# liuyuan-pal/Gen6D

Hardware: NVIDIA H100
Metric: poses/sec end-to-end (128^2 crop, 64 refs, 3 refine iters) (higher is better)
Workload: dtype f32

## Files before the change

gen6d_b200/_lib.py:

```python
import ctypes as C
import os
import re

HERE = os.path.dirname(os.path.abspath(__file__))
LIB_PATH = os.path.join(HERE, 'libgen6d_b200.so')
HEADER_PATH = os.path.join(os.path.dirname(HERE), 'include', 'gen6d_b200.h')

G6D_DET_MAX_SCALES = 8
G6D_GLUE_MAX_OBJECTS = 16
G6D_DET_MAX_INSTANCES = 16
G6D_DET_MAX_PEAK_RADIUS = 3
G6D_ATTENTION_MAX_SMEM_FLOATS = 12288 - 32
G6D_FRAMES_MAX = 1024
G6D_FRAME_RGB, G6D_FRAME_NV12 = 0, 1
PRO_NONE, PRO_AFFINE, PRO_AFFINE_RELU, PRO_CORR = 0, 1, 2, 3
ACT_NONE, ACT_RELU, ACT_LEAKY01 = 0, 1, 2
TC_TF32, TC_F16 = 0, 1
TC_PRENORM, TC_REUSE_IM2COL, TC_FOLD_SPLITS = 1, 4, 32


class ConvDesc(C.Structure):
    _fields_ = [(n, C.c_int) for n in ('B', 'D', 'H', 'W', 'Cin', 'in_cstride', 'in_coff', 'Cout', 'kd', 'kh', 'kw',
                                       'stride', 'pd', 'ph', 'pw', 'Do', 'Ho', 'Wo', 'out_cstride', 'out_coff',
                                       'prologue')] + [('group_rows', C.c_longlong), ('act', C.c_int), ('max_chain_k', C.c_int)]


class DetMaps(C.Structure):
    _fields_ = [('n_scales', C.c_int), ('rfn', C.c_int), ('hs', C.c_int), ('ws', C.c_int),
                ('map', (C.c_void_p * 3) * G6D_DET_MAX_SCALES),
                ('H', (C.c_int * 3) * G6D_DET_MAX_SCALES), ('W', (C.c_int * 3) * G6D_DET_MAX_SCALES),
                ('mu', C.c_float * 3), ('inv_sigma', C.c_float * 3), ('clip', C.c_float)]


class GlueCamera(C.Structure):
    _fields_ = [('K', C.c_double * 9), ('Kinv', C.c_double * 9), ('f', C.c_double), ('f_sq', C.c_double)]


class GlueRefs(C.Structure):
    _fields_ = [('poses', C.c_void_p), ('cen', C.c_void_p), ('f', C.c_void_p), ('dist', C.c_void_p), ('center', C.c_double * 3)]


class GlueViews(C.Structure):
    _fields_ = [('poses', C.c_void_p), ('R_look', C.c_void_p), ('RlookR', C.c_void_p), ('f', C.c_void_p), ('Kinv', C.c_void_p),
                ('src', C.c_void_p), ('rows', C.c_void_p), ('cols', C.c_void_p), ('even_idx', C.c_void_p), ('even_dirs', C.c_void_p),
                ('n_views', C.c_int), ('n_even', C.c_int), ('ref_num', C.c_int), ('size', C.c_int),
                ('norm_scale', C.c_double), ('norm_offset', C.c_float * 3), ('size_scale', C.c_float)]

# ... 136 lines not shown
```

gen6d_b200/csrc/conv_ffma.cu:

```cuda
#include "common.cuh"

namespace g6d {

struct ConvP {
    const float* x; const float* w; const float* bias; const float* ps; const float* pb;
    float* y; float* ws;
    int B, D, H, W, Cin, ics, ico, Cout, ldw, kd, kh, kw, stride, pd, ph, pw, Do, Ho, Wo, ocs, oco, pro, act;
    long long group_rows;
    int M, K, ktiles, splits, kt_per_split;
};

constexpr int BM = 128, BK = 16, NT = 256;

__device__ __forceinline__ float act_apply(float v, int act) {
    if (act == G6D_ACT_RELU) return fmaxf(v, 0.f);
    if (act == G6D_ACT_LEAKY01) return v > 0.f ? v : 0.1f * v;
    return v;
}

template <int TN>
__global__ void __launch_bounds__(NT, 2) conv_ffma_kernel(const ConvP p) {
    constexpr int BN = 16 * TN;
    constexpr int HN = BN / 2;
    constexpr int B_F4 = (BK * BN / 4);
// ... 286 lines not shown
    }
}

static int fill_params(const g6d_conv_desc* d, ConvP& p) {
    G6D_REQUIRE(d != nullptr, "g6d_conv: null desc");
    G6D_REQUIRE(d->B > 0 && d->D > 0 && d->H > 0 && d->W > 0 && d->Cin > 0 && d->Cout > 0, "g6d_conv: bad dims");
    G6D_REQUIRE(d->kd > 0 && d->kh > 0 && d->kw > 0 && d->stride > 0, "g6d_conv: bad kernel/stride");
    G6D_REQUIRE((d->Cin & 3) == 0 && (d->in_cstride & 3) == 0 && (d->in_coff & 3) == 0,
                "g6d_conv: Cin (%d), in_cstride (%d), in_coff (%d) must be multiples of 4", d->Cin, d->in_cstride,
                d->in_coff);
    G6D_REQUIRE(d->in_coff + d->Cin <= d->in_cstride, "g6d_conv: input channel slice out of row");
    G6D_REQUIRE(d->out_coff + d->Cout <= d->out_cstride, "g6d_conv: output channel slice out of row");
    const int Do = (d->D + 2 * d->pd - d->kd) / d->stride + 1;
    const int Ho = (d->H + 2 * d->ph - d->kh) / d->stride + 1;
    const int Wo = (d->W + 2 * d->pw - d->kw) / d->stride + 1;
    G6D_REQUIRE(Do == d->Do && Ho == d->Ho && Wo == d->Wo, "g6d_conv: output dims mismatch (%d,%d,%d) vs (%d,%d,%d)",
                d->Do, d->Ho, d->Wo, Do, Ho, Wo);
    G6D_REQUIRE(d->prologue >= 0 && d->prologue <= 3 && d->act >= 0 && d->act <= 2, "g6d_conv: bad prologue/act");
    if (d->prologue == G6D_PRO_AFFINE || d->prologue == G6D_PRO_AFFINE_RELU)
        G6D_REQUIRE(d->group_rows > 0, "g6d_conv: group_rows must be > 0 for affine prologue");
    const long long M = (long long)d->B * Do * Ho * Wo;
    const long long K = (long long)d->kd * d->kh * d->kw * d->Cin;
    G6D_REQUIRE(M < (1ll << 31) && K < (1ll << 31), "g6d_conv: problem too large");
    p.B = d->B; p.D = d->D; p.H = d->H; p.W = d->W; p.Cin = d->Cin; p.ics = d->in_cstride; p.ico = d->in_coff;
    p.Cout = d->Cout; p.ldw = (d->Cout + 3) & ~3; p.kd = d->kd; p.kh = d->kh; p.kw = d->kw; p.stride = d->stride;
    p.pd = d->pd; p.ph = d->ph; p.pw = d->pw; p.Do = Do; p.Ho = Ho; p.Wo = Wo; p.ocs = d->out_cstride;
    p.oco = d->out_coff; p.pro = d->prologue; p.act = d->act; p.group_rows = d->group_rows > 0 ? d->group_rows : 1;
    p.M = (int)M; p.K = (int)K; p.ktiles = (int)((K + BK - 1) / BK);
    const int bn = d->Cout > 64 ? 128 : (d->Cout > 32 ? 64 : 32);
    const long long ctas = (long long)ceil_div(M, BM) * ceil_div(d->Cout, bn);
    int splits = 1;
    if (ctas < kNumSMs && p.ktiles >= 16) {
        splits = (int)((2 * kNumSMs + ctas - 1) / ctas);
        splits = splits > p.ktiles / 8 ? p.ktiles / 8 : splits;
        splits = splits > 64 ? 64 : splits;
        splits = splits < 1 ? 1 : splits;
    }
    p.kt_per_split = (p.ktiles + splits - 1) / splits;
    p.splits = (p.ktiles + p.kt_per_split - 1) / p.kt_per_split;
    return G6D_OK;
}

}

using namespace g6d;

extern "C" long long g6d_conv_workspace_bytes(const g6d_conv_desc* desc) {
    ConvP p{};
    if (fill_params(desc, p) != G6D_OK) return -1;
    return p.splits > 1 ? (long long)p.splits * p.M * p.Cout * (long long)sizeof(float) : 0;
}

extern "C" int g6d_conv(const g6d_conv_desc* desc, const float* x, const float* w, const float* bias,
// ... 132 lines not shown
```

gen6d_b200/csrc/conv_tc.cu:

```cuda
#include <cuda_fp16.h>
#include <string.h>

#include "tc_common.cuh"

namespace g6d {

constexpr int TC_BM = 128;
constexpr int TC_PRODUCER_WARPS = 8;
constexpr int TC_CONSUMER_WARPS = 8;
constexpr int TC_THREADS = (TC_PRODUCER_WARPS + TC_CONSUMER_WARPS) * 32;
constexpr int TC_ISSUER = TC_PRODUCER_WARPS * 32;
constexpr int TC_PRODUCER_REGS = 96, TC_CONSUMER_REGS = 160;
static_assert(TC_PRODUCER_WARPS * TC_PRODUCER_REGS + TC_CONSUMER_WARPS * TC_CONSUMER_REGS <= 65536 / 32, "register file of one SM");
constexpr int TC_FOLD_PRODUCER_REGS = 40, TC_FOLD_CONSUMER_REGS = 216;
static_assert(TC_PRODUCER_WARPS * TC_FOLD_PRODUCER_REGS + TC_CONSUMER_WARPS * TC_FOLD_CONSUMER_REGS <= 65536 / 32, "register file of one SM");
static_assert(TC_BM == 64 * (TC_CONSUMER_WARPS / 4), "one 64-row wgmma tile per consumer warpgroup");
constexpr int TC_MAX_K_PER_CHAIN = 2048;

template <int KIND> struct KindCfg;
template <> struct KindCfg<G6D_TC_TF32> {
    static constexpr int BK = 32;
    static constexpr int NV = 1;
    static constexpr float CROSS = 1.f;
};
// ... 865 lines not shown
           (long long)d->D * d->H * d->W < (1ll << 30) && d->group_rows < (1ll << 31);
}

static int fill_tc_params(const g6d_conv_desc* d, int kind, ConvTcP& p) {
    G6D_REQUIRE(d != nullptr, "g6d_conv_tc: null desc");
    G6D_REQUIRE(kind == G6D_TC_TF32 || kind == G6D_TC_F16, "g6d_conv_tc: bad operand kind %d", kind);
    G6D_REQUIRE(d->B > 0 && d->D > 0 && d->H > 0 && d->W > 0 && d->Cin > 0, "g6d_conv_tc: bad dims");
    G6D_REQUIRE(d->Cout >= 16, "g6d_conv_tc: Cout (%d) must be at least 16", d->Cout);
    G6D_REQUIRE(d->kd > 0 && d->kh > 0 && d->kw > 0 && d->stride > 0, "g6d_conv_tc: bad kernel/stride");
    const int bk = kind_bk(kind);
    G6D_REQUIRE((d->Cin % bk) == 0, "g6d_conv_tc: Cin (%d) must be a multiple of %d", d->Cin, bk);
    G6D_REQUIRE((d->in_cstride & 3) == 0 && (d->in_coff & 3) == 0, "g6d_conv_tc: in_cstride/in_coff must be multiples of 4");
    G6D_REQUIRE(d->in_coff + d->Cin <= d->in_cstride, "g6d_conv_tc: input channel slice out of row");
    G6D_REQUIRE(d->out_coff + d->Cout <= d->out_cstride, "g6d_conv_tc: output channel slice out of row");
    G6D_REQUIRE(tc2_dims_ok(d), "g6d_conv_tc: spatial extent too large for the tensor-core kernel");
    const int Do = (d->D + 2 * d->pd - d->kd) / d->stride + 1;
    const int Ho = (d->H + 2 * d->ph - d->kh) / d->stride + 1;
    const int Wo = (d->W + 2 * d->pw - d->kw) / d->stride + 1;
    G6D_REQUIRE(Do > 0 && Ho > 0 && Wo > 0 && Do == d->Do && Ho == d->Ho && Wo == d->Wo, "g6d_conv_tc: output dims mismatch");
    G6D_REQUIRE(d->prologue >= 0 && d->prologue <= 3 && d->act >= 0 && d->act <= 2, "g6d_conv_tc: bad prologue/act");
    const long long M = (long long)d->B * Do * Ho * Wo;
    const long long K = (long long)d->kd * d->kh * d->kw * d->Cin;
    G6D_REQUIRE(M < (1ll << 31) && K < (1ll << 31), "g6d_conv_tc: problem too large");
    p.B = d->B; p.D = d->D; p.H = d->H; p.W = d->W; p.Cin = d->Cin; p.ics = d->in_cstride; p.ico = d->in_coff;
    p.Cout = d->Cout; p.kd = d->kd; p.kh = d->kh; p.kw = d->kw; p.stride = d->stride; p.pd = d->pd; p.ph = d->ph;
    p.pw = d->pw; p.Do = Do; p.Ho = Ho; p.Wo = Wo; p.ocs = d->out_cstride; p.oco = d->out_coff; p.pro = d->prologue;
    p.act = d->act; p.group_rows = d->group_rows > 0 ? d->group_rows : 1;
    p.M = (int)M; p.K = (int)K; p.kblocks = (int)(K / bk);
    const int bn = tc_block_n(d->Cout);
    const long long ctas = (long long)ceil_div(M, TC_BM) * ceil_div(d->Cout, bn);
    const int min_kb = 256 / bk;
    int splits = 1;
    if (ctas < kNumSMs && p.kblocks >= 2 * min_kb) {
        splits = (int)(kNumSMs / ctas);
        splits = splits > p.kblocks / min_kb ? p.kblocks / min_kb : splits;
        splits = splits < 1 ? 1 : splits;
    }
    const int nmain = tc_nmain(bn);
    const int chain = d->max_chain_k > 0 ? d->max_chain_k * nmain : (K > TC_MAX_K_PER_CHAIN ? TC_MAX_K_PER_CHAIN * nmain : 0);
    const int max_kb = chain > bk ? chain / bk : 1;
    const int min_splits = chain > 0 ? (p.kblocks + max_kb - 1) / max_kb : 1;
    splits = splits < min_splits ? min_splits : splits;
    splits = splits > 64 ? 64 : splits;
    p.kb_per_split = (p.kblocks + splits - 1) / splits;
    p.splits = (p.kblocks + p.kb_per_split - 1) / p.kb_per_split;
    return G6D_OK;
}

template <int BN, int KIND, bool FOLD, bool XR>
static int launch_tc2(const ConvTcP& p, const CUtensorMap& mh, const CUtensorMap& ml, const CUtensorMap& ma, cudaStream_t st) {
    constexpr int SMEM = XR ? Tc2XrCfg<BN>::SMEM_BYTES : Tc2Cfg<BN>::SMEM_BYTES;
    static bool configured = false;
    if (!configured) {
// ... 307 lines not shown
    const int rows = TC_BM + (d->kh - 1) * Wp + d->kw - 1;
    const int budget = 220 * 1024;
    const int b_stage = 2 * bn * 128;
    {
        const long long tiles = ((long long)Ho * Wp + TC_BM - 1) / TC_BM;
        if ((long long)Ho * Wo * 100 < tiles * TC_BM * 60) return false;
    }
    const long long a_stage = 2ll * ((rows + 7) / 8 * 8) * 128;
    const int tab_bytes = 4 * rows;
    int a_st = 2, b_st = 3;
    long long used = a_st * a_stage + b_st * b_stage + tab_bytes + 2048;
    if (used > budget) return false;
    while (b_st < 4 && used + b_stage <= budget) { ++b_st; used += b_stage; }
    while (a_st < 4 && used + a_stage <= budget) { ++a_st; used += a_stage; }
    p.B = d->B; p.D = d->D; p.H = d->H; p.W = d->W; p.Cin = d->Cin; p.ics = d->in_cstride; p.ico = d->in_coff;
    p.Cout = d->Cout; p.kd = d->kd; p.kh = d->kh; p.kw = d->kw; p.pd = d->pd; p.ph = d->ph; p.pw = d->pw;
    p.Do = Do; p.Ho = Ho; p.Wo = Wo; p.ocs = d->out_cstride; p.oco = d->out_coff; p.pro = d->prologue; p.act = d->act;
    p.group_rows = d->group_rows > 0 ? d->group_rows : 1;
    p.Wp = Wp; p.tiles_per_plane = (Ho * Wp + TC_BM - 1) / TC_BM;
    p.seg_rows = rows; p.rows_pad = (rows + 7) / 8 * 8; p.cblocks = d->Cin / kind_bk(kind);
    p.M = d->B * Do * Ho * Wo;
    p.a_stages = a_st; p.b_stages = b_st;
    *smem_bytes = (int)(a_st * a_stage) + b_st * b_stage + 256 + tab_bytes + 1024 + 64;
    const long long ctas = (long long)d->B * Do * p.tiles_per_plane * ((d->Cout + bn - 1) / bn);
    const long long K = (long long)d->Cin * d->kd * d->kh * d->kw;
    int splits = 1;
    if (ctas < kNumSMs && p.cblocks >= 2) splits = (int)((kNumSMs + ctas - 1) / ctas);
    const int nmain = tc_nmain(bn);
    const long long chain = d->max_chain_k > 0 ? (long long)d->max_chain_k * nmain : (K > TC_MAX_K_PER_CHAIN ? TC_MAX_K_PER_CHAIN * nmain : 0);
    if (chain > 0) { const int ms = (int)((K + chain - 1) / chain); splits = splits < ms ? ms : splits; }
    splits = splits > p.cblocks ? p.cblocks : splits;
    splits = splits < 1 ? 1 : splits;
    p.cb_per_split = (p.cblocks + splits - 1) / splits;
    p.splits = (p.cblocks + p.cb_per_split - 1) / p.cb_per_split;
    return true;
}

__global__ void __launch_bounds__(256) flat_moments_kernel(const float* __restrict__ y, int ocs, int oco, int Cout, int Ho, int Wo,
                                                           int Wp, int slices_per_plane, double* __restrict__ stats,
                                                           long long stats_rows) {
    __shared__ double red[8][4][4];
    const int warp = threadIdx.x >> 5, lane = threadIdx.x & 31;
    const long long m_plane = (long long)blockIdx.x * Ho * Wo;
    const int n0 = 8 * blockIdx.y + 2 * (lane & 3);
    double acc[4] = {0.0, 0.0, 0.0, 0.0};
    for (int sl = warp; sl < slices_per_plane; sl += 8) {
        const int f = sl * 16 + (lane >> 2);
// ... 327 lines not shown
```

gen6d_b200/network/selector.py:

```python
from dataclasses import dataclass

import numpy as np
import torch

from .. import ops
from .backbone import pack_vgg, vgg_v1
from .base import Branches, PackedModule, linear_as_conv
from .params import SEL_TOWER_POST, SEL_TOWERS, VGG11BNParams, selector_modules

IN_EPS = 1e-5


class LocalComm:
    rank, world, capturable = 0, 1, True

    def all_reduce_sum(self, t):
        return t

    def all_gather_cat(self, t, dim=0):
        return t

    def shard_range(self, n):
        return 0, n


FEAT_PAD = 516


@dataclass
class SelectorRefs:
    feats_cache: list
    sums: list
    pose_embed: torch.Tensor
    shape: tuple
    rfn_total: int


class ViewpointSelector(PackedModule):
    default_cfg = {'selector_angle_num': 5}

    def __init__(self, cfg):
        self.cfg = {**self.default_cfg, **cfg}
        super().__init__()
        self.backbone = VGG11BNParams()
        for name, mod in selector_modules(self.cfg['selector_angle_num']).items():
            setattr(self, name, mod)
        self.refs = None
        self.comm = LocalComm()

# ... 77 lines not shown
        x = vp.to(self.device).reshape(rfn, 1, 1, 4)
        for i, pc in enumerate(p['vpe']):
            x = ops.conv(x, pc, act=ops.ACT_RELU if i < 2 else ops.ACT_NONE)
        return SelectorRefs(feats_cache, sums, x.reshape(rfn, 512), (rfn, an), rfn_total)

    @staticmethod
    def s2_counters_for(refs, device):
        return torch.zeros(3 * refs.shape[0] * refs.shape[1], device=device, dtype=torch.int32)

    def comm_stats(self):
        return dict(getattr(self.comm, 'calls', {}))

    def _s2_counters(self):
        n = 3 * self.ref_shape[0] * self.ref_shape[1]
        c = self.__dict__.get('_s2_done')
        if c is None or c.numel() != n or c.device != self.device:
            c = torch.zeros(n, device=self.device, dtype=torch.int32)
            self.__dict__['_s2_done'] = c
        return c

    def _finalize(self, ws, rows_total):
        return ops.instnorm_finalize(self.comm.all_reduce_sum(ws), rows_total, IN_EPS)

    def _tower(self, level, ref, scale, shift, cat_buf, S, refs):
        convs = self.packed()['towers'][level]
        x, pro, ps, pb = ref, ops.PRO_CORR, scale, shift
        for i, (pc, post) in enumerate(convs):
            last = i + 1 == len(convs)
            if last:
                ops.conv(x, pc, prologue=pro, pro_scale=ps, pro_shift=pb, group_rows=S, out=cat_buf, out_coff=256 * level,
                         prenorm=True, reuse_im2col=True, fold_splits=True)
                break
            rows = x.shape[0] * x.shape[1] * x.shape[2]
            y, ws = ops.conv(x, pc, prologue=pro, pro_scale=ps, pro_shift=pb, group_rows=S, stats_rows=rows, prenorm=True,
                             reuse_im2col=True, fold_splits=True)
            ps, pb = self._finalize(ws, rows // refs.shape[0] * refs.rfn_total)
            pro = ops.PRO_AFFINE_RELU if 'r' in post else ops.PRO_AFFINE
            x = ops.maxpool2x2(y) if 'p' in post else y

    def _towers_sharded(self, q_feats, cat_buf, S, S_total, refs):
        towers = self.packed()['towers']
        nbr = 3 if self.comm.capturable else 1
        state, keep = [], []
        for l, (q, ref, (s1, s2)) in enumerate(zip(q_feats, refs.feats_cache, refs.sums)):
            h, w, c = q.shape
            scale, shift = ops.sel_corr_prologue(q.reshape(h * w, c), s1, s2, S_total, IN_EPS)
            state.append({'x': ref, 'pro': ops.PRO_CORR, 'ps': scale, 'pb': shift, 'i': 0})
        for _ in range(max(len(t) for t in towers)):
            br = Branches(nbr)
            pend = []
            for l, st in enumerate(state):
                convs = towers[l]
                if st['i'] >= len(convs):
                    continue
                pc, post = convs[st['i']]
                last = st['i'] + 1 == len(convs)

                def step(l=l, st=st, pc=pc, last=last):
                    if last:
                        ops.conv(st['x'], pc, prologue=st['pro'], pro_scale=st['ps'], pro_shift=st['pb'], group_rows=S,
                                 out=cat_buf, out_coff=256 * l, prenorm=True, reuse_im2col=True,
                                 fold_splits=True)
                        return None
                    rows = st['x'].shape[0] * st['x'].shape[1] * st['x'].shape[2]
                    return ops.conv(st['x'], pc, prologue=st['pro'], pro_scale=st['ps'], pro_shift=st['pb'], group_rows=S,
                                    stats_rows=rows, prenorm=True, reuse_im2col=True, fold_splits=True) + (rows,)
                res = br.run(l, step)
                st['i'] += 1
                if res is not None:
                    pend.append((st, post, res))
            br.join()
            if not pend:
                continue
            flat = torch.cat([ws.reshape(-1) for _, _, (_, ws, _) in pend]) if len(pend) > 1 else pend[0][2][1].reshape(-1)
            flat = self.comm.all_reduce_sum(flat)
            o = 0
            for st, post, (y, ws, rows) in pend:
                n = ws.numel()
                ps, pb = ops.instnorm_finalize(flat[o:o + n].reshape(ws.shape), rows // refs.shape[0] * refs.rfn_total, IN_EPS)
                o += n
                keep.append((y, ws))
                st['ps'], st['pb'] = ps, pb
                st['pro'] = ops.PRO_AFFINE_RELU if 'r' in post else ops.PRO_AFFINE
                st['x'] = ops.maxpool2x2(y) if 'p' in post else y

    def _select_one(self, q_feats, refs=None, counters=None):
        p = self.packed()
        if refs is None:
            refs, counters = self.refs, self._s2_counters()
        rfn, an = refs.shape
        S = rfn * an
        S_total = refs.rfn_total * an
        if counters is None or counters.numel() != 3 * S:
            raise ValueError('_select_one: a reference record other than the module\'s needs its own S2 counters [3*S]')
        dev = self.device
        cat_buf = torch.empty(S, 4, 4, 768, device=dev, dtype=torch.float32)
        feats = torch.empty(S, FEAT_PAD, device=dev, dtype=torch.float32)
        scores = ops.sel_corr_score3([r.reshape(S, -1, r.shape[-1]) for r in refs.feats_cache],
                                     [q.reshape(-1, q.shape[-1]) for q in q_feats], counters=counters)
        if self.comm.world == 1:
            br = Branches(3)
            keep = []

            def one_level(l, q, ref, s1, s2):
                h, w, c = q.shape
                scale, shift = ops.sel_corr_prologue(q.reshape(h * w, c), s1, s2, S_total, IN_EPS)
                keep.append((scale, shift))
                self._tower(l, ref, scale, shift, cat_buf, S, refs)

            for l, (q, ref, (s1, s2)) in enumerate(zip(q_feats, refs.feats_cache, refs.sums)):
                br.run(l, lambda l=l, q=q, ref=ref, s1=s1, s2=s2: one_level(l, q, ref, s1, s2))
            br.join()
        else:
            self._towers_sharded(q_feats, cat_buf, S, S_total, refs)
        y, ws = ops.conv(cat_buf, p['cf0'], stats_rows=S * 16)
        ps, pb = self._finalize(ws, S_total * 16)
        y = ops.avgpool_affine(y.reshape(S * 16, 512), 16, ps, pb, rows_per_group=S * 16, act=ops.ACT_RELU)
        ops.conv(y.reshape(S, 1, 1, 512), p['cf3'], out=feats.reshape(S, 1, 1, FEAT_PAD), out_coff=0)
        if self.comm.world == 1:
            ops.sel_vp_norm(scores, feats, 512, IN_EPS)
        else:
            all_scores = self.comm.all_gather_cat(scores, dim=1).contiguous()
            tmp = torch.empty(S_total, 4, device=dev, dtype=torch.float32)
            ops.sel_vp_norm(all_scores, tmp, 0, IN_EPS)
            r0, _ = self.comm.shard_range(refs.rfn_total)
            feats[:, 512:516] = tmp[r0 * an:r0 * an + S]
        x = ops.conv(feats.reshape(S, 1, 1, FEAT_PAD), p['sp0'], act=ops.ACT_RELU)
        x = ops.conv(x, p['sp2']).reshape(rfn, an, 512)
        sf = ops.sel_max_angle_add(x, refs.pose_embed)
        sf = self.comm.all_gather_cat(sf, dim=0).contiguous()
        rfn_local, rfn = rfn, refs.rfn_total
        for att, (m0, m3) in zip(p['atts'], p['mlps']):
            x4 = sf.reshape(rfn, 1, 1, 512)
            qv = ops.conv(x4, att['conv_query']).reshape(rfn, 512)
            kv = ops.conv(x4, att['conv_key']).reshape(rfn, 512)
            vv = ops.conv(x4, att['conv_feats']).reshape(rfn, 512)
            msg = ops.attention(qv, kv, vv, heads=8, head_major=True)
            msg = ops.conv(msg.reshape(rfn, 1, 1, 512), att['conv_merge']).reshape(rfn, 512)
            msg = ops.layernorm(msg, att['ln_w'], att['ln_b'], 1e-5)
            y = ops.conv(torch.cat([sf, msg], 1).reshape(rfn, 1, 1, 1024), m0)
            ps, pb = ops.instnorm_stats(y, rows_per_group=rfn, eps=IN_EPS)
            y = ops.conv(y, m3, prologue=ops.PRO_AFFINE_RELU, pro_scale=ps, pro_shift=pb, group_rows=rfn)
            ps, pb = ops.instnorm_stats(y, rows_per_group=rfn, eps=IN_EPS)
            y = ops.affine_act(y.reshape(rfn, 512), ps, pb, rows_per_group=rfn, act=ops.ACT_RELU)
            sf = ops.add(y, sf)
        x = ops.conv(sf.reshape(rfn, 1, 1, 512), p['score_predict'][0], act=ops.ACT_RELU)
        logits = ops.conv(x, p['score_predict'][1]).reshape(rfn)
        x = feats.reshape(rfn_local, 1, 1, an * FEAT_PAD)
        for i, pc in enumerate(p['angle_predict']):
            x = ops.conv(x, pc, act=ops.ACT_RELU if i < 2 else ops.ACT_NONE)
        angles = self.comm.all_gather_cat(x.reshape(rfn_local), dim=0)
        return logits, angles, scores

    def _select_nhwc(self, que_norm4):
        if self.ref_feats_cache is None:
            raise RuntimeError('ViewpointSelector: load_ref_imgs / extract_ref_feats must be called first')
        feats = self._feats(que_norm4)
        logits, angles, taps = [], [], []
        for qi in range(que_norm4.shape[0]):
            lg, ang, sc = self._select_one([f[qi] for f in feats])
            logits.append(lg)
            angles.append(ang)
            taps.append(sc)
        return torch.stack(logits, 0), torch.stack(angles, 0), torch.stack(taps, 0)

    def _select_u8(self, u8):
        logits, angles, _ = self._select_nhwc(ops.preprocess_u8(u8, out_c=4, imagenet_norm=True))
        idx, out = ops.sel_parse(logits, angles)
        return idx, out, logits

    def extract_ref_feats(self, ref_imgs, ref_poses, object_center, object_vert, is_train=False):
        if is_train:
            raise NotImplementedError('inference-only build: random forward-view selection is a training feature')
        with torch.no_grad():
            an, rfn, _, h, w = ref_imgs.shape
            r0, r1 = self.comm.shard_range(rfn)
            x = ref_imgs[:, r0:r1].permute(1, 0, 2, 3, 4).reshape((r1 - r0) * an, 3, h, w).float().contiguous()
            x = ops.imagenet_norm(ops.nchw_to_nhwc(x), out_c=4)
            self._load_nhwc(x, rfn, an, ref_poses, object_center, object_vert)

    def compute_view_point_feats(self, que_imgs):
        with torch.no_grad():
            x = ops.imagenet_norm(ops.nchw_to_nhwc(que_imgs.float().contiguous()), out_c=4)
            logits, angles, _ = self._select_nhwc(x)
        return logits, angles

    def forward(self, data):
# ... 59 lines not shown
```

gen6d_b200/objects.py:

```python
import numpy as np
import torch

from . import frames as F
from . import glue
from . import instances
from . import ops
from .graphs import StageCache


def require_device_pipeline(est, what):
    if est.refiner is None:
        raise ValueError(f'{what} refines every pose: the estimator needs a refiner')
    if getattr(est.selector.comm, 'world', 1) > 1:
        raise ValueError(f'{what} does not shard the selector: the estimator\'s selector is sharded over GPUs')
    if est.cfg['host_warps']:
        raise ValueError(f"{what} cuts its crops on the device: cfg['host_warps'] must be False")


class _Object:

    def __init__(self, det, sel, ref, ref_info, tables, counters, weights_gen):
        self.det, self.sel, self.ref = det, sel, ref
        self.ref_info, self.tables, self.counters = ref_info, tables, counters
        self.weights_gen = weights_gen
# ... 76 lines not shown
        o = det._detect_objects_nhwc(ops.preprocess_u8(u8, out_c=3, imagenet_norm=False), self._detector_kernels(),
                                     len(objs), objs[0].det.rfn, return_taps)
        out, _ = ops.det_parse(o['score_predict'], o['scale_predict'], o['offset_predict'], det.pool_ratio)
        return out, o

    def _initial_poses_device_fn(self, detect=None):
        est = self.est
        objs = list(self._objects.values())
        K, res = len(objs), est.cfg['ref_resolution']
        sel = est.selector

        def fn(frames, cams):
            qn = frames.shape[0]
            rows = lambda t, o: t[o * qn:(o + 1) * qn]
            cat = lambda ts: ts[0] if len(ts) == 1 else torch.cat(ts, 0)
            det = F.per_size(lambda u8: self._detect(u8)[0], frames) if detect is None else detect(frames)
            S = det.shape[0] // qn
            jobs = cat([ops.glue_detection_jobs(rows(det, s), frames, res) for s in range(S)])
            crop = ops.warp_affine_u8(jobs, S * qn, res, res)
            feats = sel._feats(ops.preprocess_u8(crop, out_c=4, imagenet_norm=True))
            poses, sels = [], []
            for s in range(S):
                ob = objs[s % K]
                lg, ang = [], []
                for qi in range(qn):
                    l, a, _ = sel._select_one([f[s * qn + qi] for f in feats], ob.sel, ob.counters)
                    lg.append(l)
                    ang.append(a)
                logits = torch.stack(lg, 0)
                idx, sel_out = ops.sel_parse(logits, torch.stack(ang, 0))
                sels.append((idx, sel_out, logits))
                poses.append(ops.glue_initial_poses(rows(det, s), idx, sel_out, ob.tables['refs'], cams))
            return cat(poses), det, sels, crop
        return fn

    def _peaks_detect_fn(self, M, radius, nms_iou, min_score):
        est = self.est
        det_mod, box = est.detector, float(est.cfg['ref_resolution'])
        objs = list(self._objects.values())
        extra = []

        def one_size(u8):
            o = det_mod._detect_objects_nhwc(ops.preprocess_u8(u8, out_c=3, imagenet_norm=False), self._detector_kernels(),
                                             len(objs), objs[0].det.rfn)
            det, _, valid, count = ops.det_parse_peaks(o['score_predict'], o['scale_predict'], o['offset_predict'], M, radius,
                                                       nms_iou, box, min_score, det_mod.pool_ratio)
            return det.reshape(-1, 4), valid.reshape(-1), count

        def detect(frames):
            det, valid, count = F.per_size(one_size, frames)
            extra[:] = [valid, count]
            return det
        return detect, extra
# ... 138 lines not shown
```

gen6d_b200/ops.py:

```python
import ctypes as C
import os
from dataclasses import dataclass
from typing import Optional

import torch

from . import _lib
from ._lib import ACT_LEAKY01, ACT_NONE, ACT_RELU, PRO_AFFINE, PRO_AFFINE_RELU, PRO_CORR, PRO_NONE


WARP_JOB_BYTES = 88


def _stream():
    return C.c_void_p(torch.cuda.current_stream().cuda_stream)


def _p(t, dtype=torch.float32):
    if t is None:
        return None
    if not (t.is_cuda and t.dtype == dtype and t.is_contiguous()):
        raise ValueError(f'expected a contiguous CUDA {dtype} tensor, got {t.dtype} {t.device} '
                         f'contiguous={t.is_contiguous()} shape={tuple(t.shape)}')
    return C.c_void_p(t.data_ptr())
# ... 487 lines not shown
        pc.w_hi = torch.empty(rows, taps * cin_pad, device=w.device, dtype=_tc_dtype(kind))
        pc.w_lo = torch.empty_like(pc.w_hi)
        _call('g6d_pack_conv_weight_tc', _p(w), _p(pc.w_hi, pc.w_hi.dtype), _p(pc.w_lo, pc.w_lo.dtype), cout, cin, cin_pad,
              taps, rows, _p(cout_scale.contiguous()) if cout_scale is not None else None, kind, _stream())
    return pc


def split_operand(x, kind=None):
    kind = tc_kind_for(x.shape[-1]) if kind is None else kind
    hi = torch.empty(x.shape, device=x.device, dtype=_tc_dtype(kind))
    lo = torch.empty_like(hi)
    _call('g6d_split_operand', _p(x), _p(hi, hi.dtype), _p(lo, lo.dtype), x.numel(), kind, _stream())
    return hi, lo, kind


def transpose_to_packed(x2d):
    rows, cols = x2d.shape
    out = torch.empty(cols, (rows + 3) // 4 * 4, device=x2d.device, dtype=torch.float32)
    _call('g6d_transpose2d', _p(x2d), _p(out), rows, cols, _stream())
    return out


def conv(x, pc, prologue=PRO_NONE, pro_scale=None, pro_shift=None, group_rows=1, act=ACT_NONE,
         in_coff=0, out=None, out_coff=0, stats_rows=None, prenorm=False, reuse_im2col=False, fold_splits=False):
    four = x.dim() == 4
    if four:
        B, H, W, cs = x.shape
        D = 1
    else:
        B, D, H, W, cs = x.shape
    kd, kh, kw = pc.k
    pd, ph, pw = pc.pad
    s = pc.stride
    Do, Ho, Wo = (D + 2 * pd - kd) // s + 1, (H + 2 * ph - kh) // s + 1, (W + 2 * pw - kw) // s + 1
    if out is None:
        shape = (B, Ho, Wo, pc.cout) if four else (B, Do, Ho, Wo, pc.cout)
        out = torch.empty(shape, device=x.device, dtype=torch.float32)
    d = _lib.ConvDesc(B=B, D=D, H=H, W=W, Cin=pc.cin, in_cstride=cs, in_coff=in_coff, Cout=pc.cout, kd=kd, kh=kh,
                      kw=kw, stride=s, pd=pd, ph=ph, pw=pw, Do=Do, Ho=Ho, Wo=Wo, out_cstride=out.shape[-1],
                      out_coff=out_coff, prologue=prologue, group_rows=group_rows, act=act, max_chain_k=pc.max_chain_k)
    work = 2.0 * B * Do * Ho * Wo * pc.cout * kd * kh * kw * pc.cin
    M = B * Do * Ho * Wo
    stats = None
    if pc.w_hi is not None and conv_path() == 'tc' and _lib.lib().g6d_conv_tc_supported(C.byref(d), pc.kind):
        flags = ((_lib.TC_PRENORM if prenorm else 0) | (_lib.TC_REUSE_IM2COL if reuse_im2col else 0)
                 | (_lib.TC_FOLD_SPLITS if fold_splits else 0))
        nbytes = _lib.lib().g6d_conv_tc_workspace_bytes_ex(C.byref(d), pc.kind, flags)
        if nbytes < 0:
            _lib.check(-1, 'g6d_conv_tc_workspace_bytes_ex')
        ws = torch.empty(nbytes // 4, device=x.device, dtype=torch.float32) if nbytes > 0 else None
        fuse = stats_rows is not None and _lib.lib().g6d_conv_tc_stats_supported(C.byref(d), pc.kind, stats_rows)
        if fuse:
            stats = torch.empty(M // stats_rows, pc.cout, 2, device=x.device, dtype=torch.float64)
        def tag(d=d, kind=pc.kind, flags=flags):
            plan = (C.c_int * 6)()
            _lib.check(_lib.lib().g6d_conv_tc_plan_v2(C.byref(d), kind, flags, plan, 6), 'g6d_conv_tc_plan_v2')
            a_op = (' prenorm' if prologue != PRO_NONE else ' im2col') if plan[3] else ''
            if flags & _lib.TC_REUSE_IM2COL and plan[3]:
                plain = (C.c_int * 4)()
                _lib.check(_lib.lib().g6d_conv_tc_plan_ex(C.byref(d), kind, flags & ~_lib.TC_REUSE_IM2COL, plain),
                           'g6d_conv_tc_plan_ex')
                a_op += '-ro' if plain[0] else ''
            a_op += '-xr' if plan[5] else ''
# ... 95 lines not shown
    s2 = torch.empty_like(s1)
    _call('g6d_sel_ref_sums', _p(ref), S, Pn, Cc, _p(s1, torch.float64), _p(s2, torch.float64), _stream())
    return s1, s2


def sel_corr_prologue(q, s1, s2, S, eps=1e-5):
    Pn, Cc = q.shape
    scale = torch.empty(Pn, Cc, device=q.device, dtype=torch.float32)
    shift = torch.empty(Cc, device=q.device, dtype=torch.float32)
    _call('g6d_sel_corr_prologue', _p(q), _p(s1, torch.float64), _p(s2, torch.float64), S, Pn, Cc, eps, _p(scale),
          _p(shift), _stream())
    return scale, shift


def sel_corr_score(ref, q, out=None):
    S, Pn, Cc = ref.shape
    if out is None:
        out = torch.empty(S, device=ref.device, dtype=torch.float32)
    _call('g6d_sel_corr_score', _p(ref), _p(q), S, Pn, Cc, _p(out), _stream(),
          work=4.0 * (S * Pn * Cc + Pn * Cc + S))
    return out


def sel_corr_score3(refs, qs, counters=None):
    S, Cc = refs[0].shape[0], refs[0].shape[2]
    Ps = [r.shape[1] for r in refs]
    out = torch.empty(3, S, device=refs[0].device, dtype=torch.float32)
    ws = torch.empty(_lib.lib().g6d_sel_corr_score3_workspace_bytes(S, *Ps) // 4, device=refs[0].device, dtype=torch.float32)
    _call('g6d_sel_corr_score3', _p(refs[0]), _p(refs[1]), _p(refs[2]), _p(qs[0]), _p(qs[1]), _p(qs[2]), S, Ps[0], Ps[1],
          Ps[2], Cc, _p(out), _p(ws), _p(counters, torch.int32), _stream(), work=4.0 * (S * sum(Ps) * Cc + sum(Ps) * Cc + 3 * S))
    return out


def sel_vp_norm(score, feats, coff, eps=1e-5):
    Ln, n = score.shape
    _call('g6d_sel_vp_norm', _p(score), Ln, n, eps, _p(feats), feats.shape[-1], coff, _stream())


def sel_max_angle_add(x, embed):
    rfn, an, Cc = x.shape
    out = torch.empty(rfn, Cc, device=x.device, dtype=torch.float32)
    _call('g6d_sel_max_angle_add', _p(x), _p(embed), _p(out), rfn, an, Cc, _stream())
    return out


def attention(q, k, v, heads, head_major=False):
    n, Cc = q.shape
    out = torch.empty_like(q)
    _call('g6d_attention_headmajor' if head_major else 'g6d_attention', _p(q), _p(k), _p(v), _p(out), n, Cc, heads, _stream())
    return out


def layernorm(x, gamma, beta, eps=1e-5):
    rows, Cc = x.shape
    out = torch.empty_like(x)
    _call('g6d_layernorm', _p(x), _p(gamma), _p(beta), _p(out), rows, Cc, eps, _stream())
    return out


def sel_parse(logits, angles):
    qn, rfn = logits.shape
    idx = torch.empty(qn, device=logits.device, dtype=torch.int64)
    out = torch.empty(qn, 2, device=logits.device, dtype=torch.float32)
    _call('g6d_sel_parse', _p(logits), _p(angles), qn, rfn, _p(idx, torch.int64), _p(out), _stream())
    return idx, out


def ref_volume_fill(ref_feats, que_feats, ref_Ks, ref_poses, que_Ks, que_poses, sn, img_h, img_w):
    Q, R, fh, fw, Cc = ref_feats.shape
    mean_in = torch.empty(Q, sn, sn, sn, 2 * Cc, device=ref_feats.device, dtype=torch.float32)
    stdv = torch.empty(Q, sn, sn, sn, Cc, device=ref_feats.device, dtype=torch.float32)
# ... 12 lines not shown
```

include/gen6d_b200.h:

```cpp
#ifndef GEN6D_B200_H
#define GEN6D_B200_H

#include <stdint.h>

#ifdef __cplusplus
extern "C" {
#endif

#define G6D_OK 0
#define G6D_EINVAL (-1)
#define G6D_ECUDA (-2)

typedef void* g6d_stream_t;

const char* g6d_last_error(void);
int g6d_version(void);
long long g6d_launch_count(void);

int g6d_preprocess_u8(const uint8_t* img, float* out, long long n_pixels, int out_c, int imagenet_norm,
                      g6d_stream_t stream);
typedef struct g6d_warp_job {
    const uint8_t* src;
    int rows, cols;
    double M[9];
// ... 152 lines not shown
                       const float* scale, const float* shift, int act, g6d_stream_t stream);
int g6d_add(const float* a, const float* b, float* out, long long n, g6d_stream_t stream);

int g6d_instnorm_stats(const float* x, long long rows, int C, int cstride, int coff, long long rows_per_group,
                       float eps, float* scale, float* shift, double* ws, g6d_stream_t stream);

int g6d_instnorm_partial(const float* x, long long rows, int C, int cstride, int coff, long long rows_per_group,
                         double* ws, g6d_stream_t stream);
int g6d_instnorm_finalize(const double* ws, long long groups, int C, long long count, float eps, float* scale,
                          float* shift, g6d_stream_t stream);

typedef struct g6d_conv_desc {
    int B, D, H, W, Cin;
    int in_cstride, in_coff;
    int Cout, kd, kh, kw;
    int stride;
    int pd, ph, pw;
    int Do, Ho, Wo;
    int out_cstride, out_coff;
    int prologue;
    long long group_rows;
    int act;
    int max_chain_k;
} g6d_conv_desc;

#define G6D_PRO_NONE 0
#define G6D_PRO_AFFINE 1
#define G6D_PRO_AFFINE_RELU 2
#define G6D_PRO_CORR 3
#define G6D_ACT_NONE 0
#define G6D_ACT_RELU 1
#define G6D_ACT_LEAKY01 2

int g6d_conv(const g6d_conv_desc* desc, const float* x, const float* w, const float* bias,
             const float* pro_scale, const float* pro_shift, float* y, void* ws, g6d_stream_t stream);
long long g6d_conv_workspace_bytes(const g6d_conv_desc* desc);
int g6d_vgg_first_block(const float* x, const float* w, const float* bias, float* y, int B, int H, int W,
                        g6d_stream_t stream);
int g6d_pack_conv_weight(const float* w, float* out, int Cout, int Cin, int Cin_pad, int taps,
                         const float* cout_scale, g6d_stream_t stream);
#define G6D_TC_TF32 0
#define G6D_TC_F16 1
int g6d_conv_tc_supported(const g6d_conv_desc* desc, int kind);
int g6d_debug_desc_shift(float* out, int shift, int mode, g6d_stream_t stream);
int g6d_conv_tc_debug(int* host_out8);
long long g6d_conv_tc_workspace_bytes(const g6d_conv_desc* desc, int kind);
// ... 82 lines not shown
```

Measured before the change: 127.6.

## Batch viewpoint selector across queries and pin conv split plans to per-query rows

Replaces the per-query selector loop with a batched path that processes up to ten queries at once. The tower, fusion, MLP, attention-projection and prediction convs now run once over the concatenated batch, while kernels tied to one query (corr score, vp norm, max-angle, attention) still loop per query. A new plan_rows descriptor field makes split-K planning use the single-query row count, so the split choice stays as before while the batched launches carry more CTAs. This is meant to cut launch count and underutilisation of small per-query convs, at the cost of larger temporary buffers and possibly fewer splits than the larger M would choose.

New measurement: 133.4 (median of 6 runs). 4.6% higher.

```diff
diff --git a/gen6d_b200/_lib.py b/gen6d_b200/_lib.py
--- a/gen6d_b200/_lib.py
+++ b/gen6d_b200/_lib.py
@@ -22,7 +22,8 @@
 class ConvDesc(C.Structure):
     _fields_ = [(n, C.c_int) for n in ('B', 'D', 'H', 'W', 'Cin', 'in_cstride', 'in_coff', 'Cout', 'kd', 'kh', 'kw',
                                        'stride', 'pd', 'ph', 'pw', 'Do', 'Ho', 'Wo', 'out_cstride', 'out_coff',
-                                       'prologue')] + [('group_rows', C.c_longlong), ('act', C.c_int), ('max_chain_k', C.c_int)]
+                                       'prologue')] + [('group_rows', C.c_longlong), ('act', C.c_int), ('max_chain_k', C.c_int),
+                                                      ('plan_rows', C.c_int)]
 
 
 class DetMaps(C.Structure):
diff --git a/gen6d_b200/csrc/conv_ffma.cu b/gen6d_b200/csrc/conv_ffma.cu
--- a/gen6d_b200/csrc/conv_ffma.cu
+++ b/gen6d_b200/csrc/conv_ffma.cu
@@ -332,13 +332,15 @@
     const long long M = (long long)d->B * Do * Ho * Wo;
     const long long K = (long long)d->kd * d->kh * d->kw * d->Cin;
     G6D_REQUIRE(M < (1ll << 31) && K < (1ll << 31), "g6d_conv: problem too large");
+    G6D_REQUIRE(d->plan_rows == 0 || (d->plan_rows > 0 && Do > 0 && Ho > 0 && Wo > 0 && d->plan_rows % ((long long)Do * Ho * Wo) == 0),
+                "g6d_conv: plan_rows (%d) must be a multiple of the %d output rows of one image", d->plan_rows, Do * Ho * Wo);
     p.B = d->B; p.D = d->D; p.H = d->H; p.W = d->W; p.Cin = d->Cin; p.ics = d->in_cstride; p.ico = d->in_coff;
     p.Cout = d->Cout; p.ldw = (d->Cout + 3) & ~3; p.kd = d->kd; p.kh = d->kh; p.kw = d->kw; p.stride = d->stride;
     p.pd = d->pd; p.ph = d->ph; p.pw = d->pw; p.Do = Do; p.Ho = Ho; p.Wo = Wo; p.ocs = d->out_cstride;
     p.oco = d->out_coff; p.pro = d->prologue; p.act = d->act; p.group_rows = d->group_rows > 0 ? d->group_rows : 1;
     p.M = (int)M; p.K = (int)K; p.ktiles = (int)((K + BK - 1) / BK);
     const int bn = d->Cout > 64 ? 128 : (d->Cout > 32 ? 64 : 32);
-    const long long ctas = (long long)ceil_div(M, BM) * ceil_div(d->Cout, bn);
+    const long long ctas = (long long)ceil_div(d->plan_rows > 0 ? d->plan_rows : M, BM) * ceil_div(d->Cout, bn);
     int splits = 1;
     if (ctas < kNumSMs && p.ktiles >= 16) {
         splits = (int)((2 * kNumSMs + ctas - 1) / ctas);
diff --git a/gen6d_b200/csrc/conv_tc.cu b/gen6d_b200/csrc/conv_tc.cu
--- a/gen6d_b200/csrc/conv_tc.cu
+++ b/gen6d_b200/csrc/conv_tc.cu
@@ -911,13 +911,16 @@
     const long long M = (long long)d->B * Do * Ho * Wo;
     const long long K = (long long)d->kd * d->kh * d->kw * d->Cin;
     G6D_REQUIRE(M < (1ll << 31) && K < (1ll << 31), "g6d_conv_tc: problem too large");
+    G6D_REQUIRE(d->plan_rows >= 0 && d->plan_rows % ((long long)Do * Ho * Wo) == 0,
+                "g6d_conv_tc: plan_rows (%d) must be a multiple of the %d output rows of one image", d->plan_rows, Do * Ho * Wo);
     p.B = d->B; p.D = d->D; p.H = d->H; p.W = d->W; p.Cin = d->Cin; p.ics = d->in_cstride; p.ico = d->in_coff;
     p.Cout = d->Cout; p.kd = d->kd; p.kh = d->kh; p.kw = d->kw; p.stride = d->stride; p.pd = d->pd; p.ph = d->ph;
     p.pw = d->pw; p.Do = Do; p.Ho = Ho; p.Wo = Wo; p.ocs = d->out_cstride; p.oco = d->out_coff; p.pro = d->prologue;
     p.act = d->act; p.group_rows = d->group_rows > 0 ? d->group_rows : 1;
     p.M = (int)M; p.K = (int)K; p.kblocks = (int)(K / bk);
     const int bn = tc_block_n(d->Cout);
-    const long long ctas = (long long)ceil_div(M, TC_BM) * ceil_div(d->Cout, bn);
+    const long long plan_m = d->plan_rows > 0 ? d->plan_rows : M;
+    const long long ctas = (long long)ceil_div(plan_m, TC_BM) * ceil_div(d->Cout, bn);
     const int min_kb = 256 / bk;
     int splits = 1;
     if (ctas < kNumSMs && p.kblocks >= 2 * min_kb) {
@@ -1271,7 +1274,8 @@
     p.M = d->B * Do * Ho * Wo;
     p.a_stages = a_st; p.b_stages = b_st;
     *smem_bytes = (int)(a_st * a_stage) + b_st * b_stage + 256 + tab_bytes + 1024 + 64;
-    const long long ctas = (long long)d->B * Do * p.tiles_per_plane * ((d->Cout + bn - 1) / bn);
+    const long long plan_b = d->plan_rows > 0 ? d->plan_rows / ((long long)Do * Ho * Wo) : d->B;
+    const long long ctas = plan_b * Do * p.tiles_per_plane * ((d->Cout + bn - 1) / bn);
     const long long K = (long long)d->Cin * d->kd * d->kh * d->kw;
     int splits = 1;
     if (ctas < kNumSMs && p.cblocks >= 2) splits = (int)((kNumSMs + ctas - 1) / ctas);
diff --git a/gen6d_b200/network/selector.py b/gen6d_b200/network/selector.py
--- a/gen6d_b200/network/selector.py
+++ b/gen6d_b200/network/selector.py
@@ -25,6 +25,7 @@
 
 
 FEAT_PAD = 516
+SEL_QUERY_CHUNK = 10
 
 
 @dataclass
@@ -148,53 +149,60 @@
     def _finalize(self, ws, rows_total):
         return ops.instnorm_finalize(self.comm.all_reduce_sum(ws), rows_total, IN_EPS)
 
-    def _tower(self, level, ref, scale, shift, cat_buf, S, refs):
+    def _tower_conv(self, level, i, st, Q, S, cat_buf):
+        pc, post = self.packed()['towers'][level][i]
+        x = st['x']
+        kw = dict(prenorm=True, reuse_im2col=True, fold_splits=True)
+        if i == 0:
+            rows = x.shape[0] * x.shape[1] * x.shape[2]
+            y = torch.empty(Q * x.shape[0], x.shape[1], x.shape[2], pc.cout, device=x.device, dtype=torch.float32)
+            ws = [ops.conv(x, pc, prologue=ops.PRO_CORR, pro_scale=st['ps'][q], pro_shift=st['pb'][q], group_rows=S,
+                           out=y[q * S:(q + 1) * S], stats_rows=rows, **kw)[1] for q in range(Q)]
+            return y, (ws[0] if Q == 1 else torch.cat(ws, 0)), rows
+        rows = x.shape[0] * x.shape[1] * x.shape[2] // Q
+        if i + 1 == len(self.packed()['towers'][level]):
+            ops.conv(x, pc, prologue=st['pro'], pro_scale=st['ps'], pro_shift=st['pb'], group_rows=S, out=cat_buf,
+                     out_coff=256 * level, plan_rows=rows, **kw)
+            return None
+        return ops.conv(x, pc, prologue=st['pro'], pro_scale=st['ps'], pro_shift=st['pb'], group_rows=S, stats_rows=rows,
+                        plan_rows=rows, **kw) + (rows,)
+
+    @staticmethod
+    def _tower_next(st, post, y, ps, pb):
+        st['ps'], st['pb'] = ps, pb
+        st['pro'] = ops.PRO_AFFINE_RELU if 'r' in post else ops.PRO_AFFINE
+        st['x'] = ops.maxpool2x2(y) if 'p' in post else y
+
+    def _tower_state(self, q, ref, s1, s2, S_total):
+        Q, h, w, c = q.shape
+        pro = [ops.sel_corr_prologue(q[i].reshape(h * w, c), s1, s2, S_total, IN_EPS) for i in range(Q)]
+        return {'x': ref, 'ps': [a for a, _ in pro], 'pb': [b for _, b in pro]}
+
+    def _tower(self, level, st, Q, cat_buf, S, refs):
         convs = self.packed()['towers'][level]
-        x, pro, ps, pb = ref, ops.PRO_CORR, scale, shift
-        for i, (pc, post) in enumerate(convs):
-            last = i + 1 == len(convs)
-            if last:
-                ops.conv(x, pc, prologue=pro, pro_scale=ps, pro_shift=pb, group_rows=S, out=cat_buf, out_coff=256 * level,
-                         prenorm=True, reuse_im2col=True, fold_splits=True)
+        for i, (_, post) in enumerate(convs):
+            res = self._tower_conv(level, i, st, Q, S, cat_buf)
+            if res is None:
                 break
-            rows = x.shape[0] * x.shape[1] * x.shape[2]
-            y, ws = ops.conv(x, pc, prologue=pro, pro_scale=ps, pro_shift=pb, group_rows=S, stats_rows=rows, prenorm=True,
-                             reuse_im2col=True, fold_splits=True)
+            y, ws, rows = res
             ps, pb = self._finalize(ws, rows // refs.shape[0] * refs.rfn_total)
-            pro = ops.PRO_AFFINE_RELU if 'r' in post else ops.PRO_AFFINE
-            x = ops.maxpool2x2(y) if 'p' in post else y
-
-    def _towers_sharded(self, q_feats, cat_buf, S, S_total, refs):
+            self._tower_next(st, post, y, ps, pb)
+
+    def _towers_sharded(self, q_feats, cat_buf, Q, S, S_total, refs):
         towers = self.packed()['towers']
         nbr = 3 if self.comm.capturable else 1
-        state, keep = [], []
-        for l, (q, ref, (s1, s2)) in enumerate(zip(q_feats, refs.feats_cache, refs.sums)):
-            h, w, c = q.shape
-            scale, shift = ops.sel_corr_prologue(q.reshape(h * w, c), s1, s2, S_total, IN_EPS)
-            state.append({'x': ref, 'pro': ops.PRO_CORR, 'ps': scale, 'pb': shift, 'i': 0})
-        for _ in range(max(len(t) for t in towers)):
+        state = [self._tower_state(q, ref, s1, s2, S_total)
+                 for q, ref, (s1, s2) in zip(q_feats, refs.feats_cache, refs.sums)]
+        keep = []
+        for i in range(max(len(t) for t in towers)):
             br = Branches(nbr)
             pend = []
             for l, st in enumerate(state):
-                convs = towers[l]
-                if st['i'] >= len(convs):
+                if i >= len(towers[l]):
                     continue
-                pc, post = convs[st['i']]
-                last = st['i'] + 1 == len(convs)
-
-                def step(l=l, st=st, pc=pc, last=last):
-                    if last:
-                        ops.conv(st['x'], pc, prologue=st['pro'], pro_scale=st['ps'], pro_shift=st['pb'], group_rows=S,
-                                 out=cat_buf, out_coff=256 * l, prenorm=True, reuse_im2col=True,
-                                 fold_splits=True)
-                        return None
-                    rows = st['x'].shape[0] * st['x'].shape[1] * st['x'].shape[2]
-                    return ops.conv(st['x'], pc, prologue=st['pro'], pro_scale=st['ps'], pro_shift=st['pb'], group_rows=S,
-                                    stats_rows=rows, prenorm=True, reuse_im2col=True, fold_splits=True) + (rows,)
-                res = br.run(l, step)
-                st['i'] += 1
+                res = br.run(l, lambda l=l, st=st: self._tower_conv(l, i, st, Q, S, cat_buf))
                 if res is not None:
-                    pend.append((st, post, res))
+                    pend.append((st, towers[l][i][1], res))
             br.join()
             if not pend:
                 continue
@@ -206,89 +214,99 @@
                 ps, pb = ops.instnorm_finalize(flat[o:o + n].reshape(ws.shape), rows // refs.shape[0] * refs.rfn_total, IN_EPS)
                 o += n
                 keep.append((y, ws))
-                st['ps'], st['pb'] = ps, pb
-                st['pro'] = ops.PRO_AFFINE_RELU if 'r' in post else ops.PRO_AFFINE
-                st['x'] = ops.maxpool2x2(y) if 'p' in post else y
-
-    def _select_one(self, q_feats, refs=None, counters=None):
-        p = self.packed()
+                self._tower_next(st, post, y, ps, pb)
+
+    def _select_batch(self, q_feats, refs=None, counters=None):
         if refs is None:
             refs, counters = self.refs, self._s2_counters()
         rfn, an = refs.shape
+        if counters is None or counters.numel() != 3 * rfn * an:
+            raise ValueError('_select_batch: a reference record other than the module\'s needs its own S2 counters [3*S]')
+        Q = q_feats[0].shape[0]
+        if Q <= SEL_QUERY_CHUNK:
+            return self._select_chunk(q_feats, refs, counters)
+        parts = [self._select_chunk([f[q0:q0 + SEL_QUERY_CHUNK] for f in q_feats], refs, counters)
+                 for q0 in range(0, Q, SEL_QUERY_CHUNK)]
+        return tuple(torch.cat(t, 0) for t in zip(*parts))
+
+    def _select_chunk(self, q_feats, refs, counters):
+        p = self.packed()
+        Q = q_feats[0].shape[0]
+        rfn, an = refs.shape
         S = rfn * an
         S_total = refs.rfn_total * an
-        if counters is None or counters.numel() != 3 * S:
-            raise ValueError('_select_one: a reference record other than the module\'s needs its own S2 counters [3*S]')
         dev = self.device
-        cat_buf = torch.empty(S, 4, 4, 768, device=dev, dtype=torch.float32)
-        feats = torch.empty(S, FEAT_PAD, device=dev, dtype=torch.float32)
-        scores = ops.sel_corr_score3([r.reshape(S, -1, r.shape[-1]) for r in refs.feats_cache],
-                                     [q.reshape(-1, q.shape[-1]) for q in q_feats], counters=counters)
+        cat_buf = torch.empty(Q * S, 4, 4, 768, device=dev, dtype=torch.float32)
+        feats = torch.empty(Q * S, FEAT_PAD, device=dev, dtype=torch.float32)
+        scores = torch.empty(Q, 3, S, device=dev, dtype=torch.float32)
+        ref_rows = [r.reshape(S, -1, r.shape[-1]) for r in refs.feats_cache]
+        for q in range(Q):
+            ops.sel_corr_score3(ref_rows, [f[q].reshape(-1, f.shape[-1]) for f in q_feats], counters=counters, out=scores[q])
         if self.comm.world == 1:
             br = Branches(3)
             keep = []
 
             def one_level(l, q, ref, s1, s2):
-                h, w, c = q.shape
-                scale, shift = ops.sel_corr_prologue(q.reshape(h * w, c), s1, s2, S_total, IN_EPS)
-                keep.append((scale, shift))
-                self._tower(l, ref, scale, shift, cat_buf, S, refs)
+                st = self._tower_state(q, ref, s1, s2, S_total)
+                keep.append(st)
+                self._tower(l, st, Q, cat_buf, S, refs)
 
             for l, (q, ref, (s1, s2)) in enumerate(zip(q_feats, refs.feats_cache, refs.sums)):
                 br.run(l, lambda l=l, q=q, ref=ref, s1=s1, s2=s2: one_level(l, q, ref, s1, s2))
             br.join()
         else:
-            self._towers_sharded(q_feats, cat_buf, S, S_total, refs)
-        y, ws = ops.conv(cat_buf, p['cf0'], stats_rows=S * 16)
+            self._towers_sharded(q_feats, cat_buf, Q, S, S_total, refs)
+        y, ws = ops.conv(cat_buf, p['cf0'], stats_rows=S * 16, plan_rows=S * 16)
         ps, pb = self._finalize(ws, S_total * 16)
-        y = ops.avgpool_affine(y.reshape(S * 16, 512), 16, ps, pb, rows_per_group=S * 16, act=ops.ACT_RELU)
-        ops.conv(y.reshape(S, 1, 1, 512), p['cf3'], out=feats.reshape(S, 1, 1, FEAT_PAD), out_coff=0)
+        y = ops.avgpool_affine(y.reshape(Q * S * 16, 512), 16, ps, pb, rows_per_group=S * 16, act=ops.ACT_RELU)
+        ops.conv(y.reshape(Q * S, 1, 1, 512), p['cf3'], out=feats.reshape(Q * S, 1, 1, FEAT_PAD), out_coff=0, plan_rows=S)
         if self.comm.world == 1:
-            ops.sel_vp_norm(scores, feats, 512, IN_EPS)
+            for q in range(Q):
+                ops.sel_vp_norm(scores[q], feats[q * S:(q + 1) * S], 512, IN_EPS)
         else:
-            all_scores = self.comm.all_gather_cat(scores, dim=1).contiguous()
-            tmp = torch.empty(S_total, 4, device=dev, dtype=torch.float32)
-            ops.sel_vp_norm(all_scores, tmp, 0, IN_EPS)
+            all_scores = self.comm.all_gather_cat(scores, dim=2).contiguous()
+            tmp = torch.empty(Q, S_total, 4, device=dev, dtype=torch.float32)
+            for q in range(Q):
+                ops.sel_vp_norm(all_scores[q], tmp[q], 0, IN_EPS)
             r0, _ = self.comm.shard_range(refs.rfn_total)
-            feats[:, 512:516] = tmp[r0 * an:r0 * an + S]
-        x = ops.conv(feats.reshape(S, 1, 1, FEAT_PAD), p['sp0'], act=ops.ACT_RELU)
-        x = ops.conv(x, p['sp2']).reshape(rfn, an, 512)
-        sf = ops.sel_max_angle_add(x, refs.pose_embed)
-        sf = self.comm.all_gather_cat(sf, dim=0).contiguous()
+            feats.reshape(Q, S, FEAT_PAD)[:, :, 512:516] = tmp[:, r0 * an:r0 * an + S]
+        x = ops.conv(feats.reshape(Q * S, 1, 1, FEAT_PAD), p['sp0'], act=ops.ACT_RELU, plan_rows=S)
+        x = ops.conv(x, p['sp2'], plan_rows=S).reshape(Q * rfn, an, 512)
+        sf = torch.empty(Q * rfn, 512, device=dev, dtype=torch.float32)
+        for q in range(Q):
+            ops.sel_max_angle_add(x[q * rfn:(q + 1) * rfn], refs.pose_embed, out=sf[q * rfn:(q + 1) * rfn])
+        sf = self.comm.all_gather_cat(sf.reshape(Q, rfn, 512), dim=1).contiguous()
         rfn_local, rfn = rfn, refs.rfn_total
+        sf = sf.reshape(Q * rfn, 512)
         for att, (m0, m3) in zip(p['atts'], p['mlps']):
-            x4 = sf.reshape(rfn, 1, 1, 512)
-            qv = ops.conv(x4, att['conv_query']).reshape(rfn, 512)
-            kv = ops.conv(x4, att['conv_key']).reshape(rfn, 512)
-            vv = ops.conv(x4, att['conv_feats']).reshape(rfn, 512)
-            msg = ops.attention(qv, kv, vv, heads=8, head_major=True)
-            msg = ops.conv(msg.reshape(rfn, 1, 1, 512), att['conv_merge']).reshape(rfn, 512)
+            x4 = sf.reshape(Q * rfn, 1, 1, 512)
+            qv = ops.conv(x4, att['conv_query'], plan_rows=rfn).reshape(Q * rfn, 512)
+            kv = ops.conv(x4, att['conv_key'], plan_rows=rfn).reshape(Q * rfn, 512)
+            vv = ops.conv(x4, att['conv_feats'], plan_rows=rfn).reshape(Q * rfn, 512)
+            msg = torch.empty_like(qv)
+            for q in range(Q):
+                r = slice(q * rfn, (q + 1) * rfn)
+                ops.attention(qv[r], kv[r], vv[r], heads=8, head_major=True, out=msg[r])
+            msg = ops.conv(msg.reshape(Q * rfn, 1, 1, 512), att['conv_merge'], plan_rows=rfn).reshape(Q * rfn, 512)
             msg = ops.layernorm(msg, att['ln_w'], att['ln_b'], 1e-5)
-            y = ops.conv(torch.cat([sf, msg], 1).reshape(rfn, 1, 1, 1024), m0)
+            y = ops.conv(torch.cat([sf, msg], 1).reshape(Q * rfn, 1, 1, 1024), m0, plan_rows=rfn)
             ps, pb = ops.instnorm_stats(y, rows_per_group=rfn, eps=IN_EPS)
-            y = ops.conv(y, m3, prologue=ops.PRO_AFFINE_RELU, pro_scale=ps, pro_shift=pb, group_rows=rfn)
+            y = ops.conv(y, m3, prologue=ops.PRO_AFFINE_RELU, pro_scale=ps, pro_shift=pb, group_rows=rfn, plan_rows=rfn)
             ps, pb = ops.instnorm_stats(y, rows_per_group=rfn, eps=IN_EPS)
-            y = ops.affine_act(y.reshape(rfn, 512), ps, pb, rows_per_group=rfn, act=ops.ACT_RELU)
+            y = ops.affine_act(y.reshape(Q * rfn, 512), ps, pb, rows_per_group=rfn, act=ops.ACT_RELU)
             sf = ops.add(y, sf)
-        x = ops.conv(sf.reshape(rfn, 1, 1, 512), p['score_predict'][0], act=ops.ACT_RELU)
-        logits = ops.conv(x, p['score_predict'][1]).reshape(rfn)
-        x = feats.reshape(rfn_local, 1, 1, an * FEAT_PAD)
+        x = ops.conv(sf.reshape(Q * rfn, 1, 1, 512), p['score_predict'][0], act=ops.ACT_RELU, plan_rows=rfn)
+        logits = ops.conv(x, p['score_predict'][1], plan_rows=rfn).reshape(Q, rfn)
+        x = feats.reshape(Q * rfn_local, 1, 1, an * FEAT_PAD)
         for i, pc in enumerate(p['angle_predict']):
-            x = ops.conv(x, pc, act=ops.ACT_RELU if i < 2 else ops.ACT_NONE)
-        angles = self.comm.all_gather_cat(x.reshape(rfn_local), dim=0)
+            x = ops.conv(x, pc, act=ops.ACT_RELU if i < 2 else ops.ACT_NONE, plan_rows=rfn_local)
+        angles = self.comm.all_gather_cat(x.reshape(Q, rfn_local), dim=1)
         return logits, angles, scores
 
     def _select_nhwc(self, que_norm4):
         if self.ref_feats_cache is None:
             raise RuntimeError('ViewpointSelector: load_ref_imgs / extract_ref_feats must be called first')
-        feats = self._feats(que_norm4)
-        logits, angles, taps = [], [], []
-        for qi in range(que_norm4.shape[0]):
-            lg, ang, sc = self._select_one([f[qi] for f in feats])
-            logits.append(lg)
-            angles.append(ang)
-            taps.append(sc)
-        return torch.stack(logits, 0), torch.stack(angles, 0), torch.stack(taps, 0)
+        return self._select_batch(self._feats(que_norm4))
 
     def _select_u8(self, u8):
         logits, angles, _ = self._select_nhwc(ops.preprocess_u8(u8, out_c=4, imagenet_norm=True))
diff --git a/gen6d_b200/objects.py b/gen6d_b200/objects.py
--- a/gen6d_b200/objects.py
+++ b/gen6d_b200/objects.py
@@ -122,13 +122,8 @@
             poses, sels = [], []
             for s in range(S):
                 ob = objs[s % K]
-                lg, ang = [], []
-                for qi in range(qn):
-                    l, a, _ = sel._select_one([f[s * qn + qi] for f in feats], ob.sel, ob.counters)
-                    lg.append(l)
-                    ang.append(a)
-                logits = torch.stack(lg, 0)
-                idx, sel_out = ops.sel_parse(logits, torch.stack(ang, 0))
+                logits, angles, _ = sel._select_batch([rows(f, s) for f in feats], ob.sel, ob.counters)
+                idx, sel_out = ops.sel_parse(logits, angles)
                 sels.append((idx, sel_out, logits))
                 poses.append(ops.glue_initial_poses(rows(det, s), idx, sel_out, ob.tables['refs'], cams))
             return cat(poses), det, sels, crop
diff --git a/gen6d_b200/ops.py b/gen6d_b200/ops.py
--- a/gen6d_b200/ops.py
+++ b/gen6d_b200/ops.py
@@ -533,7 +533,8 @@
 
 
 def conv(x, pc, prologue=PRO_NONE, pro_scale=None, pro_shift=None, group_rows=1, act=ACT_NONE,
-         in_coff=0, out=None, out_coff=0, stats_rows=None, prenorm=False, reuse_im2col=False, fold_splits=False):
+         in_coff=0, out=None, out_coff=0, stats_rows=None, prenorm=False, reuse_im2col=False, fold_splits=False,
+         plan_rows=0):
     four = x.dim() == 4
     if four:
         B, H, W, cs = x.shape
@@ -549,7 +550,8 @@
         out = torch.empty(shape, device=x.device, dtype=torch.float32)
     d = _lib.ConvDesc(B=B, D=D, H=H, W=W, Cin=pc.cin, in_cstride=cs, in_coff=in_coff, Cout=pc.cout, kd=kd, kh=kh,
                       kw=kw, stride=s, pd=pd, ph=ph, pw=pw, Do=Do, Ho=Ho, Wo=Wo, out_cstride=out.shape[-1],
-                      out_coff=out_coff, prologue=prologue, group_rows=group_rows, act=act, max_chain_k=pc.max_chain_k)
+                      out_coff=out_coff, prologue=prologue, group_rows=group_rows, act=act, max_chain_k=pc.max_chain_k,
+                      plan_rows=plan_rows)
     work = 2.0 * B * Do * Ho * Wo * pc.cout * kd * kh * kw * pc.cin
     M = B * Do * Ho * Wo
     stats = None
@@ -691,10 +693,11 @@
     return out
 
 
-def sel_corr_score3(refs, qs, counters=None):
+def sel_corr_score3(refs, qs, counters=None, out=None):
     S, Cc = refs[0].shape[0], refs[0].shape[2]
     Ps = [r.shape[1] for r in refs]
-    out = torch.empty(3, S, device=refs[0].device, dtype=torch.float32)
+    if out is None:
+        out = torch.empty(3, S, device=refs[0].device, dtype=torch.float32)
     ws = torch.empty(_lib.lib().g6d_sel_corr_score3_workspace_bytes(S, *Ps) // 4, device=refs[0].device, dtype=torch.float32)
     _call('g6d_sel_corr_score3', _p(refs[0]), _p(refs[1]), _p(refs[2]), _p(qs[0]), _p(qs[1]), _p(qs[2]), S, Ps[0], Ps[1],
           Ps[2], Cc, _p(out), _p(ws), _p(counters, torch.int32), _stream(), work=4.0 * (S * sum(Ps) * Cc + sum(Ps) * Cc + 3 * S))
@@ -706,16 +709,18 @@
     _call('g6d_sel_vp_norm', _p(score), Ln, n, eps, _p(feats), feats.shape[-1], coff, _stream())
 
 
-def sel_max_angle_add(x, embed):
+def sel_max_angle_add(x, embed, out=None):
     rfn, an, Cc = x.shape
-    out = torch.empty(rfn, Cc, device=x.device, dtype=torch.float32)
+    if out is None:
+        out = torch.empty(rfn, Cc, device=x.device, dtype=torch.float32)
     _call('g6d_sel_max_angle_add', _p(x), _p(embed), _p(out), rfn, an, Cc, _stream())
     return out
 
 
-def attention(q, k, v, heads, head_major=False):
+def attention(q, k, v, heads, head_major=False, out=None):
     n, Cc = q.shape
-    out = torch.empty_like(q)
+    if out is None:
+        out = torch.empty_like(q)
     _call('g6d_attention_headmajor' if head_major else 'g6d_attention', _p(q), _p(k), _p(v), _p(out), n, Cc, heads, _stream())
     return out
 
diff --git a/include/gen6d_b200.h b/include/gen6d_b200.h
--- a/include/gen6d_b200.h
+++ b/include/gen6d_b200.h
@@ -198,6 +198,7 @@
     long long group_rows;
     int act;
     int max_chain_k;
+    int plan_rows;
 } g6d_conv_desc;
 
 #define G6D_PRO_NONE 0
```
